# chronista-club/fleetflow

Measured on AMD Instinct MI355X. Metric: container x node evaluations/sec (FFD what-if plans, work-equivalent) + achieved GB/s % HBM roofline, higher is better.
Workload: dtype u32

## Files before the change

fleetflow_amd/csrc/fp_pipe.hip:

```cpp
#include "fp_internal.h"
#include "fp_payload.h"
#include "fp_pipe_asm.h"
#include "fp_pipe_sys.h"
#include "fp_pipe_pk.h"
#include "fp_pipe_tus.h"
#include <stdlib.h>
#include <string.h>
#include <mutex>
#include <type_traits>
#include <utility>

#ifdef FP_PIPE_STATS
__device__ unsigned long long g_pipe_stats[16 * 16];
#define STAT_ADD(w, i, v) atomicAdd(&g_pipe_stats[(w) * 16 + (i)], (unsigned long long)(v))
#define STAT_CLK() __builtin_amdgcn_s_memtime()
#define STAT_ON 1
#ifdef FP_PIPE_STATS_FINE
#define STAT_GCLK() __builtin_amdgcn_s_memtime()
#define STAT_FINE 1
#else
#define STAT_GCLK() 0ull
#define STAT_FINE 0
#endif
constexpr int TL_B = 2048;
__device__ unsigned long long g_pipe_tl[16 * TL_B * 8];
constexpr int SPAN_MAX = 4096;
__device__ unsigned long long g_stage_span[SPAN_MAX * 8];
#else
#define STAT_ADD(w, i, v) ((void)0)
#define STAT_CLK() 0ull
#define STAT_GCLK() 0ull
#define STAT_ON 0
#define STAT_FINE 0
#endif

#ifndef FP_PRIO_LEVEL
#define FP_PRIO_LEVEL 2
#endif

namespace fpp {

constexpr int K = 32;
static_assert(K == FP_BUCKETS, "fp_place.hip and the pipeline agree on the bucket count");
constexpr uint32_t END = 0x80000000u;
constexpr uint32_t CYC = 0x80000000u;
constexpr uint64_t SPIN_TICKS = 100ull * 1000 * 1000 * 60;
constexpr uint32_t MAX_G = 16;
constexpr int SPIN_MAX = 12;
constexpr int NF = 5;
constexpr uint32_t IDX_POS_MASK = (1u << 21) - 1;

struct PipeArgs {
    uint32_t C, N, scen_base, W, G, R;
    uint32_t B;
    uint32_t S;
    uint32_t lag;
    uint32_t slots;
    uint32_t bounded;
    uint32_t flush;
    uint32_t kpack;
    uint32_t publish;
    uint32_t pub_mask;
    uint32_t sys;
    uint32_t *ticket;
    uint32_t *gabort;
    uint32_t *ghead;
    uint32_t *gdata;
    uint32_t *part;
    const uint32_t *s_cpu, *s_mem, *s_req, *s_conf, *s_idx;
    uint32_t *cf, *mf;
    const uint32_t *lab;
    uint32_t *cu;
    const uint8_t *sched;
    uint32_t *assign;
    uint8_t *reason;
    uint64_t *cost;
    uint32_t *err;
    uint64_t spin_ticks;
    const uint32_t *thr;
    uint32_t prio;
    uint32_t *rng;
    uint32_t pk_mode;
};

__device__ __forceinline__ uint32_t lds_acq(uint32_t *p) {
    return __builtin_amdgcn_readfirstlane(__hip_atomic_load(p, __ATOMIC_ACQUIRE, __HIP_MEMORY_SCOPE_WORKGROUP));
}
__device__ __forceinline__ void lds_rel(uint32_t *p, uint32_t v) {
    __hip_atomic_store(p, v, __ATOMIC_RELEASE, __HIP_MEMORY_SCOPE_WORKGROUP);
}

__device__ __forceinline__ uint32_t g_ld(const uint32_t *p) {
    return __hip_atomic_load(const_cast<uint32_t *>(p), __ATOMIC_RELAXED, __HIP_MEMORY_SCOPE_AGENT);
}
__device__ __forceinline__ uint32_t g_ld_u(const uint32_t *p) {
    return __builtin_amdgcn_readfirstlane(g_ld(p));
}
__device__ __forceinline__ void g_st(uint32_t *p, uint32_t v) {
    __hip_atomic_store(p, v, __ATOMIC_RELAXED, __HIP_MEMORY_SCOPE_AGENT);
}
__device__ __forceinline__ void g_touch(const uint32_t *p) {
    (void)__hip_atomic_load(const_cast<uint32_t *>(p), __ATOMIC_RELAXED, __HIP_MEMORY_SCOPE_WAVEFRONT);
}
__device__ __forceinline__ uint32_t g_ld_w(const uint32_t *p) {
    return __hip_atomic_load(const_cast<uint32_t *>(p), __ATOMIC_RELAXED, __HIP_MEMORY_SCOPE_WAVEFRONT);
}

template <class Pred>
__device__ __forceinline__ bool spin(uint32_t *word, Pred pred, uint32_t *abort_flag, uint32_t *err,
                                     uint64_t ticks, uint32_t &iters) {
    uint32_t n = 0;
    uint64_t t0 = 0;
    while (true) {
        const uint32_t v = lds_acq(word);
        if (pred(v)) { iters += n; return true; }
        if (lds_acq(abort_flag)) return false;
        if ((++n & 1023u) == 0) {
            const uint64_t now = __builtin_amdgcn_s_memrealtime();
            if (!t0) {
                t0 = now;
            } else if (now - t0 > ticks) {
                lds_rel(abort_flag, 1u);
                if ((threadIdx.x & 63) == 0) atomicMax(err, (uint32_t)(-FP_EDEVICE));
                return false;
            }
        }
        if (n < 8) __builtin_amdgcn_s_sleep(1);
        else if (n < 32) __builtin_amdgcn_s_sleep(4);
        else __builtin_amdgcn_s_sleep(SPIN_MAX);
    }
}


__device__ __forceinline__ uint32_t bucket_of(uint32_t v, uint32_t my_t, int base) {
    uint32_t k = 0;
#pragma unroll
    for (uint32_t step = K / 2; step; step >>= 1) {
        const uint32_t t = (uint32_t)__shfl((int)my_t, (int)(base + k + step));
        k += t <= v ? step : 0u;
    }
    return k;
}

__device__ __forceinline__ uint32_t fpp_rank(uint64_t m) {
    return __builtin_amdgcn_mbcnt_hi((uint32_t)(m >> 32), __builtin_amdgcn_mbcnt_lo((uint32_t)m, 0u));
}

__device__ __forceinline__ uint32_t wave_min(uint32_t v) {
    v = min(v, (uint32_t)__builtin_amdgcn_update_dpp(-1, (int)v, 0x111, 0xF, 0xF, false));
    v = min(v, (uint32_t)__builtin_amdgcn_update_dpp(-1, (int)v, 0x112, 0xF, 0xF, false));
    v = min(v, (uint32_t)__builtin_amdgcn_update_dpp(-1, (int)v, 0x114, 0xF, 0xF, false));
    v = min(v, (uint32_t)__builtin_amdgcn_update_dpp(-1, (int)v, 0x118, 0xF, 0xF, false));
    v = min(v, (uint32_t)__builtin_amdgcn_update_dpp(-1, (int)v, 0x142, 0xA, 0xF, false));
    v = min(v, (uint32_t)__builtin_amdgcn_update_dpp(-1, (int)v, 0x143, 0xC, 0xF, false));
    return __builtin_amdgcn_readlane(v, 63);
}


constexpr size_t LCTL = 64;

__device__ __forceinline__ bool gring_wait(uint32_t *tail, uint32_t need, uint32_t slots, uint32_t &seen,
                                           const PipeArgs &a, uint32_t *abort_flag, uint32_t lane,
                                           uint32_t &iters) {
    if (need - seen <= slots) return true;
    uint32_t n = 0;
    uint64_t t0 = 0;
    while (true) {
        seen = g_ld_u(tail);
        if (need - seen <= slots) { iters += n; return true; }
        if (g_ld_u(a.gabort) || lds_acq(abort_flag)) return false;
        if ((++n & 255u) == 0) {
            const uint64_t now = __builtin_amdgcn_s_memrealtime();
            if (!t0) {
                t0 = now;
            } else if (now - t0 > a.spin_ticks) {
                g_st(a.gabort, 1u);
                lds_rel(abort_flag, 1u);
                if (lane == 0) atomicMax(a.err, (uint32_t)(-FP_EDEVICE));
                return false;
            }
        }
        if (n < 8) __builtin_amdgcn_s_sleep(2);
        else __builtin_amdgcn_s_sleep(SPIN_MAX);
    }
}

template <uint32_t G>
using RecT = uint32_t[G];

#ifndef FPP_PF_MAX_WIDE
#define FPP_PF_MAX_WIDE 0
#endif
#ifndef FPP_PF_MAX_NARROW
#define FPP_PF_MAX_NARROW 4
#endif
constexpr uint32_t PF_MAX_NARROW = FPP_PF_MAX_NARROW, PF_MAX_WIDE = FPP_PF_MAX_WIDE;
#ifndef FPP_IB
#define FPP_IB 1
#endif
#ifndef FPP_IB1024
#define FPP_IB1024 1
#endif
#ifndef FPP_LOOKAHEAD
#define FPP_LOOKAHEAD 3
#endif
#ifndef FPP_DIRECT_TICKETS
#define FPP_DIRECT_TICKETS 1
#endif
constexpr uint32_t SYS_MAX_G = 4;
#ifndef FPP_MASK_UPKEEP
#define FPP_MASK_UPKEEP 0
#endif
#ifndef FPP_BIGP_NOMASK
#define FPP_BIGP_NOMASK 1
#endif
#ifndef FPP_BIGP_WAVES
#define FPP_BIGP_WAVES 7
#endif
constexpr uint32_t BIGP_WV = 7;
constexpr bool is_bigp(uint32_t G, uint32_t BLK, uint32_t WV, bool PK) {
    return G == 12 && BLK == 64 && WV == BIGP_WV && PK;
}
#ifndef FPP_PK_SYS_MAX_G
#define FPP_PK_SYS_MAX_G 4
#endif
constexpr uint32_t PK_SYS_MAX_G = FPP_PK_SYS_MAX_G;
template <uint32_t G, bool UPD, bool IB, bool PK, uint32_t... gs, class Rec>
__device__ __forceinline__ void fpp_groups(std::integer_sequence<uint32_t, gs...>, uint32_t &nxt, uint64_t &placed,
                                           uint32_t &asg, uint32_t &used, uint32_t &used_hi, Rec &rcf, Rec &rmf,
                                           Rec &rcu, const Rec &rlab, uint32_t cpu, uint32_t mem, uint32_t req,
                                           uint32_t conf, uint32_t cand, uint32_t cand_hi, uint32_t my_t, uint32_t lane,
                                           uint64_t *Mw, uint32_t mlane, uint32_t gb64, uint32_t qc, uint32_t qm, uint32_t &nchk,
                                           uint32_t &nhit, uint32_t sys, unsigned long long (&gst)[4], uint32_t cw,
                                           uint32_t qw, uint32_t sc_c, uint32_t sc_m) {
    constexpr uint32_t pf_max = G <= SYS_MAX_G ? PF_MAX_NARROW : PF_MAX_WIDE;
    (
        [&] {
            uint64_t q = __builtin_amdgcn_ballot_w64(nxt == gs);
            if (pf_max > 0 && q) {
                uint64_t e;
                if constexpr (PK) e = __builtin_amdgcn_ballot_w64(pk_fits(rcf[gs], qw));
                else e = (__builtin_amdgcn_ballot_w64(rcf[gs] >= qc) & __builtin_amdgcn_ballot_w64(rmf[gs] >= qm));
                if (__builtin_popcountll(e) <= pf_max) {
                    bool ok = false;
                    while (e) {
                        const uint32_t l = (uint32_t)__builtin_ctzll(e);
                        e &= e - 1;
                        const uint32_t nlb = __builtin_amdgcn_readlane(rlab[gs], l);
                        const uint32_t ncu = __builtin_amdgcn_readlane(rcu[gs], l);
                        if constexpr (PK) {
                            const uint32_t nw = __builtin_amdgcn_readlane(rcf[gs], l);
                            ok |= ((((nw - cw) & PK_GUARD) | (req & nlb) | (conf & ncu)) == 0u);
                        } else {
                            const uint32_t ncf = __builtin_amdgcn_readlane(rcf[gs], l);
                            const uint32_t nmf = __builtin_amdgcn_readlane(rmf[gs], l);
                            ok |= (ncf >= cpu) & (nmf >= mem) & (((req & nlb) | (conf & ncu)) == 0u);
                        }
                    }
                    const uint64_t fit = q & __builtin_amdgcn_ballot_w64(ok);
                    if (q != fit) {
                        const uint64_t above = (((uint64_t)cand_hi << 32) | cand) & ~((2ull << gs) - 1ull);
                        const uint32_t nx = above ? (uint32_t)__builtin_ctzll(above) : G;
                        nxt = ((q & ~fit) >> lane) & 1ull ? nx : nxt;
                    }
                    q = fit;
                }
            }
            if (q) {
                uint64_t touched = 0;
                const unsigned long long gc0 = STAT_GCLK();
                if constexpr (PK) {
                    if (G <= PK_SYS_MAX_G && sys && (uint32_t)__builtin_popcountll(q) >= (sys & 0xFFFFu))
                        fpp_group_sysp<gs, G>(q, placed, touched, asg, nxt, rcf[gs], rcu[gs], rlab[gs], cw, req, conf,
                                              cand, cand_hi, gb64, nchk, nhit, qw, sys >> 16);
                    else
                        fpp_group_xp<gs, G, IB>(q, placed, touched, asg, nxt, rcf[gs], rcu[gs], rlab[gs], cw, req, conf,
                                                cand, cand_hi, gb64, nchk, nhit, qw);
                } else {
                    if (G <= SYS_MAX_G && sys && (uint32_t)__builtin_popcountll(q) >= (sys & 0xFFFFu))
                        fpp_group_sys<gs, G>(q, placed, touched, asg, nxt, rcf[gs], rmf[gs], rcu[gs], rlab[gs], cpu, mem,
                                             req, conf, cand, cand_hi, gb64, nchk, nhit, qc, qm, sys >> 16);
                    else
                        fpp_group_x<gs, G, IB>(q, placed, touched, asg, nxt, rcf[gs], rmf[gs], rcu[gs], rlab[gs], cpu, mem,
                                               req, conf, cand, cand_hi, gb64, nchk, nhit, qc, qm);
                }
                const unsigned long long gc1 = STAT_GCLK();
                if (STAT_FINE) { gst[0] += gc1 - gc0; gst[2] += 1; gst[3] += (uint32_t)__builtin_popcountll(touched); }
                if (touched) {
                    auto node_cm = [&](uint32_t l, uint32_t &nc, uint32_t &nm) {
                        if constexpr (PK) {
                            const uint32_t nw = __builtin_amdgcn_readlane(rcf[gs], l);
                            nc = pk_cpu(nw, sc_c);
                            nm = pk_mem(nw, sc_m);
                        } else {
                            nc = __builtin_amdgcn_readlane(rcf[gs], l);
                            nm = __builtin_amdgcn_readlane(rmf[gs], l);
                        }
                    };
                    if constexpr (IB) {
                        if (gs < 32) used = fpp_lane_sel<true>(touched, used | (1u << gs), used);
                        else used_hi = fpp_lane_sel<true>(touched, used_hi | (1u << (gs & 31)), used_hi);
                        if (UPD) {
                            uint32_t clr_lo = 0, clr_hi = 0;
                            uint64_t tt = touched;
                            while (tt) {
                                const uint32_t l = (uint32_t)__builtin_ctzll(tt);
                                tt &= tt - 1;
                                uint32_t nc, nm;
                                node_cm(l, nc, nm);
                                const uint64_t below = (__builtin_amdgcn_ballot_w64(my_t > nc) & 0xFFFFFFFFull) |
                                                       (__builtin_amdgcn_ballot_w64(my_t > nm) & ~0xFFFFFFFFull);
                                if (l < 32) clr_lo = fpp_lane_sel<true>(below, clr_lo | (1u << l), clr_lo);
                                else clr_hi = fpp_lane_sel<true>(below, clr_hi | (1u << (l & 31)), clr_hi);
                            }
                            const uint64_t clr = ((uint64_t)clr_hi << 32) | clr_lo;
                            if (__builtin_amdgcn_ballot_w64(clr != 0))
                                asm volatile("ds_and_b64 %0, %1 offset:%2" ::"v"(mlane), "v"(~clr),
                                             "i"(gs * K * 2 * 8) : "memory");
                        }
                    } else {
                        const bool me = (touched >> lane) & 1ull;
                        if (gs < 32) used |= me ? (1u << gs) : 0u;
                        else used_hi |= me ? (1u << (gs & 31)) : 0u;
                        if (UPD) {
                            uint64_t clr = 0, tt = touched;
                            while (tt) {
                                const uint32_t l = (uint32_t)__builtin_ctzll(tt);
                                tt &= tt - 1;
                                uint32_t nc, nm;
                                node_cm(l, nc, nm);
                                clr |= (my_t > (lane < 32 ? nc : nm)) ? (1ull << l) : 0ull;
                            }
                            if (__builtin_amdgcn_ballot_w64(clr != 0))
                                atomicAnd((unsigned long long *)&Mw[(size_t)gs * K * 2 + (lane & (K - 1)) * 2 + (lane >> 5)],
                                          ~clr);
                        }
                    }
                }
                if (STAT_FINE) gst[1] += STAT_GCLK() - gc1;
            }
        }(),
        ...);
}

constexpr uint32_t WIDE_WAVES = 3, WIDE12_WAVES = 5;
#ifndef FPP_BIG_WAVES
#define FPP_BIG_WAVES 6
#endif
#ifndef FPP_BIG_S
#define FPP_BIG_S 4096
#endif
[[maybe_unused]] constexpr uint32_t WIDE12_BIG_WAVES = FPP_BIG_WAVES, WIDE12_BIG_S = FPP_BIG_S;
template <uint32_t G, uint32_t BLK, uint32_t WV = 0, bool PK = false>
__global__ __launch_bounds__(BLK, BLK == 64 ? (is_bigp(G, BLK, WV, PK) ? FPP_BIGP_WAVES
                                                : WV   ? WV
                                                : G == 12 ? WIDE12_WAVES
                                                          : WIDE_WAVES)
                                               : 1) void
k_ffd_pipe(const PipeArgs a_arg) {
#if defined(__HIP_DEVICE_COMPILE__)
    const PipeArgs &a = *(const PipeArgs *)__builtin_amdgcn_kernarg_segment_ptr();
#else
    const PipeArgs &a = a_arg;
#endif
    extern __shared__ __attribute__((aligned(16))) unsigned char smem[];
#ifndef FPP_W1
#define FPP_W1 1
#endif
    constexpr bool one_wave = BLK == 64 && FPP_W1;
    const uint32_t W = one_wave ? 1u : a.W, R = a.R, B = a.B, prio = a.prio;
    const uint32_t w = one_wave ? 0u : __builtin_amdgcn_readfirstlane(threadIdx.x >> 6);
    const uint32_t lane = threadIdx.x & 63;
    const uint32_t C = a.C, N = a.N;
    const uint32_t pmask = a.kpack ? IDX_POS_MASK : ~CYC;
    using GM = typename std::conditional<(G > 32), uint64_t, uint32_t>::type;

    constexpr bool NM = is_bigp(G, BLK, WV, PK) && FPP_BIGP_NOMASK;
    uint64_t *M = reinterpret_cast<uint64_t *>(smem);
    uint32_t *CTL = reinterpret_cast<uint32_t *>(M + (NM ? 0 : (size_t)W * G * K * 2));
    uint32_t *CNT = CTL + (W - 1) * 8;
    uint32_t *D = CNT + 8;

    uint32_t sc_c = 0, sc_m = 0;
    if (PK || a.pk_mode) {
        const uint32_t orc = __builtin_amdgcn_readfirstlane(a.rng[0]), orm = __builtin_amdgcn_readfirstlane(a.rng[1]);
        sc_c = orc ? (uint32_t)__builtin_ctz(orc) : 0u;
        sc_m = orm ? (uint32_t)__builtin_ctz(orm) : 0u;
        const bool packs = (orc >> sc_c) <= PK_FIELD_MAX && (orm >> sc_m) <= PK_FIELD_MAX;
        if (packs != PK) return;
    }
    if (blockIdx.x == 0 && threadIdx.x == 0 && a.rng) a.rng[2] = PK ? 2u : 1u;
    for (uint32_t i = threadIdx.x; i < (W - 1) * 8 + 8; i += blockDim.x) CTL[i] = 0;
    __syncthreads();
    if (threadIdx.x == 0) {
        const uint32_t total = (a.S + (B - 1) * a.lag) * B;
        uint32_t t;
        if (FPP_DIRECT_TICKETS && a.lag == a.S) {
            const uint32_t v = atomicAdd(a.ticket, 1u);
            t = v < a.S * B ? v * B + v / a.S : 0xFFFFFFFFu;
        } else {
            while (true) {
                t = atomicAdd(a.ticket, 1u);
                if (t >= total) { t = 0xFFFFFFFFu; break; }
                const uint32_t r = t / B, bb = t % B;
                if (r >= bb * a.lag && r - bb * a.lag < a.S) break;
            }
        }
        CNT[4] = t;
    }
    __syncthreads();
    const uint32_t tk = __builtin_amdgcn_readfirstlane(CNT[4]);
    if (tk == 0xFFFFFFFFu) return;
    const uint32_t b = tk % B, s = tk / B - b * a.lag;
    const size_t cb = (size_t)s * C, nb = (size_t)s * N;

    static_assert(K == 32, "mask/threshold lane layout assumes K == 32");
    const uint32_t my_t = NM ? 0u : a.thr[lane];
    const uint32_t gbase = (b * W + w) * G;
    uint64_t *Mw = M + (size_t)w * G * K * 2;
    const uint32_t mlane = (uint32_t)(uintptr_t)(__attribute__((address_space(3))) uint64_t *)(Mw + (lane & (K - 1)) * 2 + (lane >> 5));
    RecT<G> rcf, rmf, rcu, rlab;
    GM schedbits = 0;
    uint32_t usedbits = 0, used_hi = 0;
    {
        const uint32_t n0 = gbase * 64 + lane;
        const uint32_t *cf0 = a.cf + nb + n0, *mf0 = a.mf + nb + n0, *cu0 = a.cu + nb + n0, *lb0 = a.lab + nb + n0;
        const uint8_t *sc0 = a.sched + nb + n0;
#pragma unroll
        for (uint32_t g = 0; g < G; ++g) {
            const bool in = n0 + g * 64 < N;
            const int o = in ? (int)(g * 64) : -(int)n0;
            const bool sc = in && sc0[o] != 0;
            const uint32_t x = cf0[o], y = mf0[o], z = cu0[o], l = lb0[o];
            if constexpr (PK) {
                rcf[g] = sc ? pk_pack(x, y, sc_c, sc_m) : 0u;
            } else {
                rcf[g] = sc ? x : 0u;
                rmf[g] = sc ? y : 0u;
            }
            rcu[g] = sc ? z : 0xFFFFFFFFu;
            rlab[g] = sc ? ~l : 0xFFFFFFFFu;
            schedbits |= sc ? (GM(1) << g) : GM(0);
        }
    }
    uint32_t zs_g = G, zs_l = 0;
#pragma unroll
    for (uint32_t g = 0; g < G; ++g) {
        const uint64_t sm = __builtin_amdgcn_ballot_w64(((schedbits >> g) & 1u) != 0);
        if (zs_g == G && sm) {
            zs_g = g;
            zs_l = (uint32_t)__builtin_ctzll(sm);
        }
    }
#pragma unroll 1
    for (uint32_t k = 0; k < (NM ? 0u : (uint32_t)K); ++k) {
        const uint32_t tc = __builtin_amdgcn_readlane(my_t, k), tm = __builtin_amdgcn_readlane(my_t, K + k);
#pragma unroll
        for (uint32_t g = 0; g < G; ++g) {
            const bool sc = (schedbits >> g) & 1u;
            const uint32_t ncf = PK ? pk_cpu(rcf[g], sc_c) : rcf[g], nmf = PK ? pk_mem(rcf[g], sc_m) : rmf[g];
            const uint64_t bc = __builtin_amdgcn_ballot_w64(sc & (ncf >= tc));
            const uint64_t bm = __builtin_amdgcn_ballot_w64(sc & (nmf >= tm));
            if (lane == k) {
                Mw[((size_t)g * K + k) * 2] = bc;
                Mw[((size_t)g * K + k) * 2 + 1] = bm;
            }
        }
    }
    __syncthreads();

    const bool has_out = w + 1 < W;
    const bool g_in = w == 0 && b > 0;
    const bool g_out = w + 1 == W && b + 1 < B;
    const size_t LSLOT = 2 * 64;
    uint32_t *gin_head = a.ghead + ((size_t)s * (B - 1) + (b - 1)) * LCTL;
    uint32_t *gin_data = a.gdata + ((size_t)s * (B - 1) + (b - 1)) * a.slots * LSLOT;
    uint32_t *gout_head = a.ghead + ((size_t)s * (B - 1) + b) * LCTL;
    uint32_t *gout_data = a.gdata + ((size_t)s * (B - 1) + b) * a.slots * LSLOT;
    constexpr bool unbounded_only = BLK == 64 && WV != 0;
    const uint32_t gslots = a.slots, gbounded = unbounded_only ? 0u : a.bounded;
    const uint32_t gflush = unbounded_only ? (a.flush & 1u) : a.flush;
#define GSLOT(i) (unbounded_only ? (uint32_t)(i) : (uint32_t)(i) % gslots)
    uint32_t otail_seen = 0;
    uint32_t *octl = CTL + w * 8;
    uint32_t *ictl = CTL + (w - 1) * 8;
    uint32_t *odata = D + (size_t)w * R * NF * 64;
    uint32_t *idata = D + (size_t)(w - 1) * R * NF * 64;
    uint32_t *abort_flag = &CNT[2];
    uint32_t ohead = 0, ofill = 0, itail = 0, k0 = 0;
    uint32_t ihead_seen = 0;
    constexpr uint32_t LA = BLK == 64 ? (FPP_LOOKAHEAD >= 3 ? 1 : FPP_LOOKAHEAD) : 0;
    [[maybe_unused]] uint32_t la_n = 0, la_pos = 0;
    [[maybe_unused]] bool la_ok = false;
    constexpr bool DB = BLK == 64 && G == 12 && PK && FPP_LOOKAHEAD >= 3, DB_EARLY = DB && FPP_LOOKAHEAD == 3;
    [[maybe_unused]] uint32_t nf_cpu = 0, nf_mem = 0, nf_req = 0, nf_conf = 0, nf_idx = 0, nf_n = 0;
    [[maybe_unused]] bool nf_ok = false;
    [[maybe_unused]] uint32_t la2_n = 0, la2_pos = 0;
    constexpr int VMCNT0 = 0x0F70;
#define FPP_REQUEST_NEXT()                                                                              \
    do {                                                                                                \
        uint32_t off_;                                                                                  \
        if (g_in) {                                                                                     \
            const uint32_t tn_ = __builtin_amdgcn_readfirstlane(la_n);                                  \
            off_ = (la_ok && !(tn_ & END) && lane < tn_) ? la_pos & pmask : 0u;                         \
            nf_n = tn_;                                                                                 \
            nf_ok = la_ok;                                                                              \
        } else {                                                                                        \
            off_ = min(k0 + lane, C - 1u);                                                              \
            nf_ok = true;                                                                               \
        }                                                                                               \
        const size_t o_ = cb + off_;                                                                    \
        nf_cpu = g_ld_w(a.s_cpu + o_);                                                                  \
        nf_mem = g_ld_w(a.s_mem + o_);                                                                  \
        nf_req = g_ld_w(a.s_req + o_);                                                                  \
        nf_conf = g_ld_w(a.s_conf + o_);                                                                \
        if (!g_in) nf_idx = g_ld_w(a.s_idx + o_);                                                       \
        else if (!DB_EARLY) nf_idx = la_pos;                                                            \
        if (DB_EARLY && g_in) {  \
            la_ok = itail + 1u < ihead_seen;                                                            \
            const uint32_t *sn_ = la_ok ? gin_data + (size_t)GSLOT(itail + 1u) * LSLOT : a.s_idx + cb;  \
            la2_n = g_ld(sn_);                                                                          \
            la2_pos = g_ld(sn_ + (la_ok ? 64u + lane : 0u));                                            \
        }                                                                                               \
    } while (0)
    uint32_t opend = 0;
    uint32_t n_used = 0, n_rej = 0;
    uint32_t st_spin_in = 0, st_spin_out = 0, st_visits = 0, st_checks = 0, st_hits = 0, st_batches = 0;
    unsigned long long ck_in = 0, ck_pre = 0, ck_cand = 0, ck_fwd = 0, ck_wait = 0, ck_gx = 0, ck_gu = 0;
    uint32_t st_queues = 0, st_touched = 0;
    const unsigned long long ck_t0 = STAT_CLK();
    unsigned long long ck_a, ck_b;
#ifdef FP_PIPE_STATS
    const unsigned long long sp_start = __builtin_amdgcn_s_memrealtime();
    unsigned long long sp_first = 0;
#endif
    bool alive = true;
    if constexpr (DB) __builtin_amdgcn_s_waitcnt(VMCNT0);
    while (alive) {
        if (prio == 2u) __builtin_amdgcn_s_setprio(0);
        ck_a = STAT_CLK();
#ifdef FP_PIPE_STATS
        const unsigned long long tl_top = ck_a;
        unsigned long long tl_avail = ck_a;
#endif
        uint32_t cpu = 0, mem = 0, req = 0, conf = 0, idx = 0;
        bool valid = false;
        if (g_in) {
            uint32_t n_sp = 0;
            uint64_t t0 = 0;
            bool got = itail < ihead_seen;
            while (!got) {
                ihead_seen = g_ld_u(gin_head);
                if (ihead_seen > itail) { got = true; break; }
                if (g_ld_u(a.gabort) || lds_acq(abort_flag)) break;
                if ((++n_sp & 255u) == 0) {
                    const uint64_t now = __builtin_amdgcn_s_memrealtime();
                    if (!t0) {
                        t0 = now;
                    } else if (now - t0 > a.spin_ticks) {
                        g_st(a.gabort, 1u);
                        lds_rel(abort_flag, 1u);
                        if (lane == 0) atomicMax(a.err, (uint32_t)(-FP_EDEVICE));
                        break;
                    }
                }
                if (n_sp < 8) __builtin_amdgcn_s_sleep(2);
                else __builtin_amdgcn_s_sleep(SPIN_MAX);
            }
            st_spin_in += n_sp;
            if (!got) break;
#ifdef FP_PIPE_STATS
            tl_avail = STAT_CLK();
#endif
            __builtin_amdgcn_fence(__ATOMIC_ACQUIRE, "wavefront");
            if (((gflush & 2u) || (gbounded && (itail & 3u) == 0)) && lane == 0) g_st(gin_head + LCTL / 2, itail);
            const uint32_t *sd = gin_data + (size_t)GSLOT(itail) * LSLOT;
            uint32_t n, pos;
            if (DB && nf_ok) {
                n = nf_n;
                pos = nf_idx;
            } else if (LA && !DB_EARLY && la_ok) {
                n = __builtin_amdgcn_readfirstlane(la_n);
                pos = la_pos;
            } else {
                n = g_ld_u(sd);
                pos = g_ld(sd + 64 + lane);
                if constexpr (NM) __builtin_amdgcn_s_waitcnt(VMCNT0);
            }
            if (n & END) break;
            valid = lane < n;
            if (DB && nf_ok) {
                idx = valid ? pos : 0u;
                cpu = valid ? nf_cpu : 0u;
                mem = valid ? nf_mem : 0u;
                req = valid ? nf_req : 0u;
                conf = valid ? nf_conf : 0u;
            } else {
                if (valid) {
                    idx = pos;
                    const uint32_t p = pos & pmask;
                    cpu = a.s_cpu[cb + p];
                    mem = a.s_mem[cb + p];
                    req = a.s_req[cb + p];
                    conf = a.s_conf[cb + p];
                }
                if constexpr (DB) __builtin_amdgcn_s_waitcnt(VMCNT0);
            }
            itail++;
        } else if (w == 0) {
            if (k0 >= C) break;
            const uint32_t i = k0 + lane;
            valid = i < C;
            if (DB && nf_ok) {
                cpu = valid ? nf_cpu : 0u;
                mem = valid ? nf_mem : 0u;
                req = valid ? nf_req : 0u;
                conf = valid ? nf_conf : 0u;
                idx = valid ? nf_idx : 0u;
            } else {
                if (valid) {
                    cpu = a.s_cpu[cb + i];
                    mem = a.s_mem[cb + i];
                    req = a.s_req[cb + i];
                    conf = a.s_conf[cb + i];
                    idx = a.s_idx[cb + i];
                }
                if constexpr (DB) __builtin_amdgcn_s_waitcnt(VMCNT0);
            }
            const bool cyc = valid && (idx & CYC);
            if (cyc) {
                const uint32_t j = idx & pmask;
                a.assign[cb + j] = FP_NONE;
                a.reason[cb + j] = (uint8_t)req;
            }
            n_rej += (uint32_t)__popcll(__ballot(cyc));
            valid = valid && !cyc;
            k0 += 64;
            if constexpr (LA >= 2) {
                if (k0 < C) {
                    const size_t ti = cb + min(k0 + (lane == 0 ? 0u : lane == 1 ? 32u : 63u), C - 1);
                    g_touch(a.s_cpu + ti);
                    g_touch(a.s_mem + ti);
                    g_touch(a.s_req + ti);
                    g_touch(a.s_conf + ti);
                    g_touch(a.s_idx + ti);
                }
            }
        } else {
            const uint32_t want = itail;
            if (!spin(&ictl[0], [want](uint32_t h) { return h != want; }, abort_flag, a.err, a.spin_ticks, st_spin_in)) break;
#ifdef FP_PIPE_STATS
            tl_avail = STAT_CLK();
#endif
            const uint32_t slot = itail % R;
            const uint32_t n = __builtin_amdgcn_readfirstlane(ictl[2 + slot]);
            if (n & END) break;
            const uint32_t *sd = idata + (size_t)slot * NF * 64;
            valid = lane < n;
            if (valid) {
                cpu = sd[lane];
                mem = sd[64 + lane];
                req = sd[128 + lane];
                conf = sd[192 + lane];
                idx = sd[256 + lane];
            }
            itail++;
            lds_rel(&ictl[1], itail);
        }
        if constexpr (LA != 0 && !DB_EARLY) {
            la_ok = g_in && itail < ihead_seen;
            if (g_in) {
                const uint32_t *sn = la_ok ? gin_data + (size_t)GSLOT(itail) * LSLOT : a.s_idx + cb;
                la_n = g_ld(sn);
                la_pos = g_ld(sn + (la_ok ? 64u + lane : 0u));
            }
        }
        uint32_t tail_async = 0;
        const bool tail_issued = (gflush & 2u) && g_out && ofill != 0;
        if (tail_issued) tail_async = g_ld(gout_head + LCTL / 2);
        uint32_t kc, km;
        if constexpr (NM) {
            kc = km = 0;
        } else if (a.kpack) {
            kc = (idx >> 21) & (uint32_t)(K - 1);
            km = (idx >> 26) & (uint32_t)(K - 1);
        } else {
            kc = bucket_of(cpu, my_t, 0);
            km = bucket_of(mem, my_t, K);
        }
        if (prio == 2u) __builtin_amdgcn_s_setprio(FP_PRIO_LEVEL);
        ck_b = STAT_CLK(); ck_in += ck_b - ck_a; ck_a = ck_b;
#ifdef FP_PIPE_STATS
        if (!sp_first) sp_first = __builtin_amdgcn_s_memrealtime();
#endif
#ifdef FP_PIPE_STATS
        const unsigned long long ck_t0_batch = ck_b;
#endif

        const uint64_t vm = __builtin_amdgcn_ballot_w64(valid);
        const uint32_t qc = vm ? __builtin_amdgcn_readlane(cpu, 63 - __builtin_clzll(vm)) : 0xFFFFFFFFu;
        const uint32_t qm = wave_min(valid ? mem : 0xFFFFFFFFu);
        const uint32_t cw = PK ? pk_pack(cpu, mem, sc_c, sc_m) : 0u;
        const uint32_t qw = PK ? pk_pack(qc, qm, sc_c, sc_m) : 0u;
        [[maybe_unused]] bool zero_early = false;
        if constexpr (DB_EARLY) {
            zero_early = valid && (cpu | mem | req | conf) == 0u;
            FPP_REQUEST_NEXT();
        }
        const uint32_t oc = kc * 2, om = km * 2 + 1;
        constexpr bool prescan_skip = G > SYS_MAX_G;
        GM cand = 0;
#pragma unroll
        for (uint32_t g = 0; g < G; ++g) {
            const uint64_t e = PK ? __builtin_amdgcn_ballot_w64(pk_fits(rcf[g], qw))
                                  : (__builtin_amdgcn_ballot_w64(rcf[g] >= qc) & __builtin_amdgcn_ballot_w64(rmf[g] >= qm));
            const uint64_t *mg = Mw + (size_t)g * K * 2;
            if constexpr (NM) {
                cand |= e ? GM(1) << g : GM(0);
            } else if (prescan_skip) {
                if (e) cand |= (mg[oc] & mg[om] & e) ? GM(1) << g : GM(0);
            } else {
                cand |= (mg[oc] & mg[om] & e) ? GM(1) << g : GM(0);
            }
        }
        cand = valid ? cand : GM(0);
        if constexpr (LA >= 2) {
            if (g_in && la_ok) {
                const uint32_t tn = __builtin_amdgcn_readfirstlane(la_n);
                if (!(tn & END)) {
                    const uint32_t tp = lane < tn ? la_pos & pmask : 0u;
                    g_touch(a.s_cpu + cb + tp);
                    g_touch(a.s_mem + cb + tp);
                    g_touch(a.s_req + cb + tp);
                    g_touch(a.s_conf + cb + tp);
                }
            }
        }
        const bool zero = DB_EARLY ? zero_early : valid && (cpu | mem | req | conf) == 0u;
        uint64_t todo = __builtin_amdgcn_ballot_w64(cand != 0 && !zero);
        uint64_t placed = 0;
        uint32_t my_assign = FP_NONE;
        if (STAT_ON) {
            st_batches++;
            st_visits += (uint32_t)__popcll(__ballot(valid));
        }
        ck_b = STAT_CLK(); ck_pre += ck_b - ck_a; ck_a = ck_b;
#ifdef FP_PIPE_STATS
        const unsigned long long tl_pre = ck_b;
        const uint32_t tl_checks0 = st_checks, tl_hits0 = st_hits, tl_todo = (uint32_t)__popcll(todo);
#endif
        {
            uint32_t nxt = ((todo >> lane) & 1ull) ? (cand ? (uint32_t)__builtin_ctzll((uint64_t)cand) : G) : G;
            uint32_t nchk = 0, nhit = 0;
            unsigned long long gst[4] = {0, 0, 0, 0};
            if (prio == 1u && todo) __builtin_amdgcn_s_setprio(FP_PRIO_LEVEL);
            if (todo)
                fpp_groups<G, (G > 1) && FPP_MASK_UPKEEP, (BLK == 64 || (FPP_IB1024 && G > SYS_MAX_G)) && FPP_IB, PK>(std::make_integer_sequence<uint32_t, G>{}, nxt, placed, my_assign, usedbits,
                                       used_hi, rcf, rmf, rcu, rlab, cpu, mem, req, conf, (uint32_t)cand,
                                       (uint32_t)((uint64_t)cand >> 32), my_t, lane, Mw, mlane,
                                       __builtin_amdgcn_readfirstlane(gbase * 64u), qc, qm, nchk, nhit, a.sys, gst,
                                       cw, qw, sc_c, sc_m);
            if (prio == 1u && todo) __builtin_amdgcn_s_setprio(0);
            if (STAT_ON) { st_checks += nchk; st_hits += nhit; }
            if (STAT_FINE) { ck_gx += gst[0]; ck_gu += gst[1]; st_queues += (uint32_t)gst[2]; st_touched += (uint32_t)gst[3]; }
        }
        if (zs_g < G) {
            const uint64_t zm = __builtin_amdgcn_ballot_w64(zero);
            if (zm) {
                placed |= zm;
                my_assign = zero ? (gbase + zs_g) * 64 + zs_l : my_assign;
                if (zs_g < 32) usedbits |= lane == zs_l ? (1u << zs_g) : 0u;
                else used_hi |= lane == zs_l ? (1u << (zs_g & 31)) : 0u;
            }
        }
        ck_b = STAT_CLK(); ck_cand += ck_b - ck_a; ck_a = ck_b;
#ifdef FP_PIPE_STATS
        const unsigned long long tl_cand = ck_b;
        const uint32_t tl_idx = st_batches - 1;
#endif
        if constexpr (DB_EARLY) {
            asm volatile("" : "+v"(nf_cpu), "+v"(nf_mem), "+v"(nf_req), "+v"(nf_conf), "+v"(nf_idx), "+v"(la2_n),
                         "+v"(la2_pos));
            if (g_in) {
                nf_idx = la_pos;
                la_n = la2_n;
                la_pos = la2_pos;
            }
        } else if constexpr (DB) {
            FPP_REQUEST_NEXT();
        }
        if ((placed >> lane) & 1ull) a.assign[cb + (idx & pmask)] = my_assign;
#ifdef FP_PIPE_STATS
        if (s == 0 && lane == 0 && tl_idx < (uint32_t)TL_B && b * W + w < 16) {
            unsigned long long *tl = &g_pipe_tl[((size_t)(b * W + w) * TL_B + tl_idx) * 8];
            tl[0] = tl_top; tl[1] = tl_avail; tl[2] = ck_t0_batch; tl[3] = tl_pre; tl[4] = tl_cand;
            tl[5] = st_checks - tl_checks0; tl[6] = st_hits - tl_hits0;
            tl[7] = tl_todo | ((unsigned long long)__popcll(vm) << 32);
        }
#endif
        const bool fwd = valid && !((placed >> lane) & 1ull);
        if (g_out) {
            const uint64_t fm = __builtin_amdgcn_ballot_w64(fwd);
            const uint32_t f = (uint32_t)__popcll(fm);
            if (f) {
                const uint32_t pos = ofill + fpp_rank(fm);
                if (gbounded &&
                    !gring_wait(gout_head + LCTL / 2, ohead + 2, gslots, otail_seen, a, abort_flag, lane, st_spin_out)) {
                    alive = false;
                    break;
                }
                if (fwd) {
                    uint32_t *sd = gout_data + (size_t)GSLOT(ohead + (pos >= 64 ? 1 : 0)) * LSLOT;
                    g_st(sd + 64 + (pos & 63u), idx);
                }
                if (ofill + f >= 64) {
                    if (lane == 0) g_st(gout_data + (size_t)GSLOT(ohead) * LSLOT, 64u);
                    ohead++;
                    if (unbounded_only ? (ohead & a.pub_mask) == 0 : ++opend >= a.publish) {
                        asm volatile("s_waitcnt vmcnt(0)" ::: "memory");
                        if (lane == 0) g_st(gout_head, ohead);
                        opend = 0;
                    }
                    ofill = ofill + f - 64;
                } else {
                    ofill += f;
                }
            }
            if (tail_issued && ofill && __builtin_amdgcn_readfirstlane(tail_async) + 1u >= ohead) {
                if (lane == 0) g_st(gout_data + (size_t)GSLOT(ohead) * LSLOT, ofill);
                asm volatile("s_waitcnt vmcnt(0)" ::: "memory");
                ohead++;
                if (lane == 0) g_st(gout_head, ohead);
                ofill = 0;
                opend = 0;
            }
            if (STAT_FINE) { ck_b = STAT_GCLK(); ck_fwd += ck_b - ck_a; }
            continue;
        }
        if (!has_out) {
            if (fwd) {
                a.assign[cb + (idx & pmask)] = FP_NONE;
                a.reason[cb + (idx & pmask)] = FP_REASON_NOFIT;
            }
            n_rej += (uint32_t)__popcll(__ballot(fwd));
            continue;
        }
        const uint64_t fm = __ballot(fwd);
        const uint32_t f = (uint32_t)__popcll(fm);
        if (f) {
            const uint32_t pos = ofill + fpp_rank(fm);
            uint32_t *od = odata + (size_t)(ohead % R) * NF * 64;
            if (fwd && pos < 64) {
                od[pos] = cpu; od[64 + pos] = mem; od[128 + pos] = req; od[192 + pos] = conf; od[256 + pos] = idx;
            }
            if (ofill + f >= 64) {
                octl[2 + ohead % R] = 64;
                ohead++;
                lds_rel(&octl[0], ohead);
                const uint32_t h = ohead;
                ck_b = STAT_CLK(); ck_fwd += ck_b - ck_a; ck_a = ck_b;
                if (!spin(&octl[1], [h, R](uint32_t tl) { return h - tl < R; }, abort_flag, a.err, a.spin_ticks, st_spin_out)) {
                    alive = false;
                    break;
                }
                ck_b = STAT_CLK(); ck_wait += ck_b - ck_a; ck_a = ck_b;
                od = odata + (size_t)(ohead % R) * NF * 64;
                if (fwd && pos >= 64) {
                    const uint32_t p = pos - 64;
                    od[p] = cpu; od[64 + p] = mem; od[128 + p] = req; od[192 + p] = conf; od[256 + p] = idx;
                }
                ofill = ofill + f - 64;
            } else {
                ofill += f;
            }
        }
        if ((gflush & 1u) && ofill && lds_acq(&octl[1]) == ohead) {
            octl[2 + ohead % R] = ofill;
            ohead++;
            lds_rel(&octl[0], ohead);
            const uint32_t h = ohead;
            if (!spin(&octl[1], [h, R](uint32_t tl) { return h - tl < R; }, abort_flag, a.err, a.spin_ticks, st_spin_out)) {
                alive = false;
                break;
            }
            ofill = 0;
        }
    }

#ifdef FP_PIPE_STATS
    if (s == 0 && lane == 0 && b * W + w < (uint32_t)SPAN_MAX) {
        unsigned long long *sp = &g_stage_span[(size_t)(b * W + w) * 8];
        sp[0] = sp_start; sp[1] = sp_first; sp[2] = __builtin_amdgcn_s_memrealtime();
        sp[3] = ck_pre + ck_cand; sp[4] = st_batches; sp[5] = ck_wait; sp[6] = st_spin_in; sp[7] = st_hits;
    }
#endif
    if (g_out && !lds_acq(abort_flag) &&
        (!gbounded || gring_wait(gout_head + LCTL / 2, ohead + 2, gslots, otail_seen, a, abort_flag, lane, st_spin_out))) {
        if (ofill) {
            if (lane == 0) g_st(gout_data + (size_t)GSLOT(ohead) * LSLOT, ofill);
            asm volatile("s_waitcnt vmcnt(0)" ::: "memory");
            ohead++;
            if (lane == 0) g_st(gout_head, ohead);
        }
        if (lane == 0) g_st(gout_data + (size_t)GSLOT(ohead) * LSLOT, END);
        asm volatile("s_waitcnt vmcnt(0)" ::: "memory");
        ohead++;
        if (lane == 0) g_st(gout_head, ohead);
    }
    if (has_out && !lds_acq(abort_flag)) {
        bool ok = true;
        if (ofill) {
            octl[2 + ohead % R] = ofill;
            ohead++;
            lds_rel(&octl[0], ohead);
            const uint32_t h = ohead;
            ok = spin(&octl[1], [h, R](uint32_t tl) { return h - tl < R; }, abort_flag, a.err, a.spin_ticks, st_spin_out);
        }
        if (ok) {
            octl[2 + ohead % R] = END;
            ohead++;
            lds_rel(&octl[0], ohead);
        }
    }
    if (G == 1) {
        const uint32_t n = gbase * 64 + lane;
        if (n < N && (schedbits & 1u) &&
            ((PK ? (a.cf[nb + n] != pk_cpu(rcf[0], sc_c) || a.mf[nb + n] != pk_mem(rcf[0], sc_m))
                 : (a.cf[nb + n] != rcf[0] || a.mf[nb + n] != rmf[0])) ||
             a.cu[nb + n] != rcu[0]))
            usedbits |= 1u;
    }
    {
        uint32_t u = (uint32_t)__popc(usedbits) + (uint32_t)__popc(used_hi);
#pragma unroll
        for (int o = 32; o > 0; o >>= 1) u += (uint32_t)__shfl_xor((int)u, o);
        n_used = u;
    }
    if (lane == 0) {
        const uint32_t st_slot = (B * W <= 16u) ? b * W + w : w;
        (void)st_slot;
        atomicAdd(&CNT[0], n_used);
        atomicAdd(&CNT[1], n_rej);
        STAT_ADD(st_slot, 0, st_visits); STAT_ADD(st_slot, 1, st_checks); STAT_ADD(st_slot, 2, st_hits);
        STAT_ADD(st_slot, 3, st_batches); STAT_ADD(st_slot, 4, st_spin_in); STAT_ADD(st_slot, 5, st_spin_out);
        STAT_ADD(st_slot, 8, ck_in); STAT_ADD(st_slot, 9, ck_pre); STAT_ADD(st_slot, 10, ck_cand); STAT_ADD(st_slot, 11, ck_fwd);
        STAT_ADD(st_slot, 12, ck_wait); STAT_ADD(st_slot, 13, STAT_CLK() - ck_t0);
        STAT_ADD(st_slot, 6, ck_gx); STAT_ADD(st_slot, 7, ck_gu); STAT_ADD(st_slot, 14, st_queues);
        STAT_ADD(st_slot, 15, st_touched);
    }
    (void)ck_t0; (void)ck_in; (void)ck_pre; (void)ck_cand; (void)ck_fwd; (void)ck_wait; (void)ck_gx; (void)ck_gu;
    (void)st_queues; (void)st_touched;
    (void)st_spin_in; (void)st_spin_out; (void)st_visits; (void)st_checks; (void)st_hits; (void)st_batches;
#undef GSLOT
#pragma unroll
    for (uint32_t g = 0; g < G; ++g) {
        const uint32_t n = (gbase + g) * 64 + lane;
        if (n < N && ((schedbits >> g) & 1u)) {
            a.cf[nb + n] = PK ? pk_cpu(rcf[g], sc_c) : rcf[g];
            a.mf[nb + n] = PK ? pk_mem(rcf[g], sc_m) : rmf[g];
            a.cu[nb + n] = rcu[g];
        }
    }
    __syncthreads();
    if (threadIdx.x == 0) {
        a.part[((size_t)s * B + b) * 2] = CNT[0];
        a.part[((size_t)s * B + b) * 2 + 1] = CNT[1];
    }
}

__global__ void k_cost_reduce(uint32_t S, uint32_t B, uint32_t scen_base, const uint32_t *__restrict__ part,
                              uint64_t *__restrict__ cost) {
    const uint32_t s = blockIdx.x * blockDim.x + threadIdx.x;
    if (s >= S) return;
    uint32_t used = 0, rej = 0;
    for (uint32_t b = 0; b < B; ++b) {
        used += part[((size_t)s * B + b) * 2];
        rej += part[((size_t)s * B + b) * 2 + 1];
    }
    cost[s] = fpd::pack_cost(rej, used, scen_base + s);
}

template <bool SUMM, bool RANGE>
__global__ __launch_bounds__(256) void k_node_summary(uint32_t N, const uint32_t *__restrict__ cf,
                                                      const uint32_t *__restrict__ mf, const uint32_t *__restrict__ lab,
                                                      const uint32_t *__restrict__ cu,
                                                      const uint8_t *__restrict__ sched, uint32_t *__restrict__ summ,
                                                      uint32_t *__restrict__ rng) {
    const size_t nb = (size_t)blockIdx.x * N;
    uint32_t u = 0, a = 0xFFFFFFFFu, oc = 0, om = 0;
    constexpr uint32_t NS_U = 4;
    for (uint32_t n0 = threadIdx.x; n0 < N; n0 += NS_U * blockDim.x) {
        uint32_t l[NS_U], c[NS_U], x[NS_U], y[NS_U];
        uint8_t sc[NS_U];
#pragma unroll
        for (uint32_t k = 0; k < NS_U; ++k) {
            const uint32_t n = n0 + k * blockDim.x;
            sc[k] = n < N ? sched[nb + n] : 0;
            if (SUMM) {
                l[k] = n < N ? lab[nb + n] : 0u;
                c[k] = n < N ? cu[nb + n] : 0xFFFFFFFFu;
            }
            if (RANGE) {
                x[k] = n < N ? cf[nb + n] : 0u;
                y[k] = n < N ? mf[nb + n] : 0u;
            }
        }
#pragma unroll
        for (uint32_t k = 0; k < NS_U; ++k) {
            if (sc[k]) {
                if (SUMM) {
                    u |= l[k];
                    a &= c[k];
                }
                if (RANGE) {
                    oc |= x[k];
                    om |= y[k];
                }
            }
        }
    }
    for (int o = 32; o > 0; o >>= 1) {
        u |= (uint32_t)__shfl_xor((int)u, o);
        a &= (uint32_t)__shfl_xor((int)a, o);
        oc |= (uint32_t)__shfl_xor((int)oc, o);
        om |= (uint32_t)__shfl_xor((int)om, o);
    }
    __shared__ uint32_t red[4][4];
    const uint32_t w = threadIdx.x >> 6;
    if ((threadIdx.x & 63) == 0) { red[0][w] = u; red[1][w] = a; red[2][w] = oc; red[3][w] = om; }
    __syncthreads();
    if (threadIdx.x == 0) {
        for (uint32_t q = 1; q < blockDim.x / 64; ++q) { u |= red[0][q]; a &= red[1][q]; oc |= red[2][q]; om |= red[3][q]; }
        if (SUMM) {
            summ[(size_t)blockIdx.x * 4] = u;
            summ[(size_t)blockIdx.x * 4 + 1] = a;
        }
        if (RANGE) {
            fp_or_new_bits(&rng[0], oc);
            fp_or_new_bits(&rng[1], om);
        }
    }
}

__device__ __forceinline__ bool screened(const uint32_t *sm, uint32_t req, uint32_t conf) {
    return ((req & ~sm[0]) | (conf & sm[1])) != 0u;
}

template <class KeyT>
__global__ void k_gather_sorted(const uint32_t *__restrict__ thr, uint32_t kpack, uint32_t S, uint32_t C,
                                const uint32_t *__restrict__ order,
                                const KeyT *__restrict__ skeys, uint32_t mbits, uint64_t cmax, uint64_t mmax,
                                const uint32_t *__restrict__ cval, const uint32_t *__restrict__ mval,
                                const uint32_t *__restrict__ cpu, const uint32_t *__restrict__ mem,
                                const uint32_t *__restrict__ req, const uint32_t *__restrict__ conf,
// ... 764 lines not shown
```

Measured before the change: 79160 billion.

## Add lazy per-group walk for no-mask big-PK path, skipping candidate prescan

For the no-mask (NM) configuration, replaces the upfront per-group candidate prescan with a lazy walk over groups that checks the wave-wide fit ballot only when lanes remain unplaced, and stops once all lanes are placed. It avoids evaluating all G groups' fit ballots before the placement loop and drops the per-lane next-group bookkeeping. A CLOSE mode (the default) also sets the query word to a guard value once nothing remains. The walk order is fixed group by group, so lanes needing late groups still visit every earlier group, and the todo mask now includes lanes that have no candidate.

Result: faster. 82080 billion, median of 6 (+3.7%).

```diff
diff --git a/fleetflow_amd/csrc/fp_pipe.hip b/fleetflow_amd/csrc/fp_pipe.hip
--- a/fleetflow_amd/csrc/fp_pipe.hip
+++ b/fleetflow_amd/csrc/fp_pipe.hip
@@ -216,6 +216,9 @@
 #endif
 #ifndef FPP_BIGP_WAVES
 #define FPP_BIGP_WAVES 7
+#endif
+#ifndef FPP_BIGP_LAZY
+#define FPP_BIGP_LAZY 2
 #endif
 constexpr uint32_t BIGP_WV = 7;
 constexpr bool is_bigp(uint32_t G, uint32_t BLK, uint32_t WV, bool PK) {
@@ -343,6 +346,42 @@
         ...);
 }
 
+template <uint32_t g, bool CLOSE>
+__device__ __forceinline__ void fpp_group_lazy_p(uint64_t &remaining, uint32_t &asg, uint32_t &used, uint32_t &rw,
+                                                 uint32_t &rcu, uint32_t rlab, uint32_t cw, uint32_t req,
+                                                 uint32_t conf, uint32_t gb64, uint32_t &nchk, uint32_t &nhit,
+                                                 unsigned long long (&gst)[4], uint32_t &qw) {
+    if (!CLOSE && !remaining) return;
+    if (!__builtin_amdgcn_ballot_w64(pk_fits(rw, qw))) return;
+    uint64_t touched = 0;
+    const unsigned long long gc0 = STAT_GCLK();
+    fpp_refilter_loop_p(remaining, touched, asg, rw, rcu, rlab, cw, req, conf, gb64 + g * 64u, nchk, qw);
+    const uint64_t hit = remaining & __builtin_amdgcn_ballot_w64(asg != 0xFFFFFFFFu);
+#ifdef FP_PIPE_STATS
+    nhit += (uint32_t)__builtin_popcountll(hit);
+#else
+    (void)nhit;
+#endif
+    remaining = fpp_uniform64(remaining & ~hit);
+    if (CLOSE) qw = remaining ? qw : PK_GUARD;
+    const unsigned long long gc1 = STAT_GCLK();
+    if (STAT_FINE) { gst[0] += gc1 - gc0; gst[2] += 1; gst[3] += (uint32_t)__builtin_popcountll(touched); }
+    if (touched) used = fpp_lane_sel<true>(touched, used | (1u << g), used);
+    if (STAT_FINE) gst[1] += STAT_GCLK() - gc1;
+}
+
+template <uint32_t G, uint32_t... gs, class Rec>
+__device__ __forceinline__ void fpp_groups_lazy(std::integer_sequence<uint32_t, gs...>, uint64_t &remaining,
+                                                uint32_t &asg, uint32_t &used, Rec &rcf, Rec &rcu, const Rec &rlab,
+                                                uint32_t req, uint32_t conf, uint32_t gb64, uint32_t &nchk,
+                                                uint32_t &nhit, unsigned long long (&gst)[4], uint32_t cw,
+                                                uint32_t qw) {
+    static_assert(G <= 32, "used bits of the lazy walk: one word");
+    (fpp_group_lazy_p<gs, FPP_BIGP_LAZY == 2>(remaining, asg, used, rcf[gs], rcu[gs], rlab[gs], cw, req, conf, gb64,
+                                              nchk, nhit, gst, qw),
+     ...);
+}
+
 constexpr uint32_t WIDE_WAVES = 3, WIDE12_WAVES = 5;
 #ifndef FPP_BIG_WAVES
 #define FPP_BIG_WAVES 6
@@ -709,9 +748,10 @@
         }
         const uint32_t oc = kc * 2, om = km * 2 + 1;
         constexpr bool prescan_skip = G > SYS_MAX_G;
+        constexpr bool LZ = NM && FPP_BIGP_LAZY;
         GM cand = 0;
 #pragma unroll
-        for (uint32_t g = 0; g < G; ++g) {
+        for (uint32_t g = 0; g < (LZ ? 0u : G); ++g) {
             const uint64_t e = PK ? __builtin_amdgcn_ballot_w64(pk_fits(rcf[g], qw))
                                   : (__builtin_amdgcn_ballot_w64(rcf[g] >= qc) & __builtin_amdgcn_ballot_w64(rmf[g] >= qm));
             const uint64_t *mg = Mw + (size_t)g * K * 2;
@@ -737,7 +777,9 @@
             }
         }
         const bool zero = DB_EARLY ? zero_early : valid && (cpu | mem | req | conf) == 0u;
-        uint64_t todo = __builtin_amdgcn_ballot_w64(cand != 0 && !zero);
+        uint64_t todo;
+        if constexpr (LZ) todo = __builtin_amdgcn_ballot_w64(valid && !zero);
+        else todo = __builtin_amdgcn_ballot_w64(cand != 0 && !zero);
         uint64_t placed = 0;
         uint32_t my_assign = FP_NONE;
         if (STAT_ON) {
@@ -749,7 +791,21 @@
         const unsigned long long tl_pre = ck_b;
         const uint32_t tl_checks0 = st_checks, tl_hits0 = st_hits, tl_todo = (uint32_t)__popcll(todo);
 #endif
-        {
+        if constexpr (LZ) {
+            uint32_t nchk = 0, nhit = 0;
+            unsigned long long gst[4] = {0, 0, 0, 0};
+            if (prio == 1u && todo) __builtin_amdgcn_s_setprio(FP_PRIO_LEVEL);
+            if (todo) {
+                uint64_t remaining = todo;
+                fpp_groups_lazy<G>(std::make_integer_sequence<uint32_t, G>{}, remaining, my_assign, usedbits,
+                                   rcf, rcu, rlab, req, conf, __builtin_amdgcn_readfirstlane(gbase * 64u), nchk, nhit,
+                                   gst, cw, qw);
+                placed = todo & ~remaining;
+            }
+            if (prio == 1u && todo) __builtin_amdgcn_s_setprio(0);
+            if (STAT_ON) { st_checks += nchk; st_hits += nhit; }
+            if (STAT_FINE) { ck_gx += gst[0]; ck_gu += gst[1]; st_queues += (uint32_t)gst[2]; st_touched += (uint32_t)gst[3]; }
+        } else {
             uint32_t nxt = ((todo >> lane) & 1ull) ? (cand ? (uint32_t)__builtin_ctzll((uint64_t)cand) : G) : G;
             uint32_t nchk = 0, nhit = 0;
             unsigned long long gst[4] = {0, 0, 0, 0};
```
